# graphcore-research/bess-kge

Measured on AMD Instinct MI355X. Metric: positive+negative triples scored/sec, higher is better.
Workload: dtype f32; 1 GPU; ogbl-biokg-shaped ComplEx d=256 fp32 (W=512), 93,773 entities per shard, n_shard=1, S=4096 positives x 256 per-triple negatives per GPU per step, EmbeddingMoving, mode=score (gather+score+loss); negatives_per_triple=256, mode=score, collectives=none

## Files before the change

bess-kge_amd/csrc/neg_pertriple.hip:

```cpp
#include "common.h"
#include "loss_rows.h"

namespace bess {

struct NegPtArgs {
    const float* query;
    const void* base;
    const int32_t* idx;
    int64_t n_query;
    int n_neg;
    int W;
    int nch;
    int nb;
    int items_per_query;
    float sign;
    int accum = 0;
    float p = 2.f;
    int dn_by_row = 0;
    int sweep_shift = -1;
};

struct FuseArgs {
    const float* pos;
    int kind;
    float beta;
    float margin;
    float shift;
    float* st_ml;
    float* st_acc;
    const uint8_t* mask = nullptr;
    int64_t mask_rows = 0;
    int mask_cols = 0, mask_from = 0;
};

__device__ __forceinline__ float sigmoid_f(float x) { return 1.f / (1.f + expf(-x)); }

template <typename T, int VEC, int IT, int RED, int UNROLL, bool FUSE>
__global__ __launch_bounds__(256) void k_neg_pertriple_fwd(NegPtArgs a, float* __restrict__ out,
                                                           int64_t ld_out, FuseArgs f) {
    const int lane = threadIdx.x & 63;
    const int g = lane & 15;
    const int sub = lane >> 4;
    const int64_t item = blockIdx.x * 4ll + (threadIdx.x >> 6);
    if (item >= a.n_query * a.items_per_query) return;
    const int64_t q = item / a.items_per_query;
    const int k0 = static_cast<int>(item - q * a.items_per_query) * a.nb;
    const int k1 = min(k0 + a.nb, a.n_neg);

    float qv[IT][VEC];
    const float* qp = a.query + q * a.W;
#pragma unroll
    for (int it = 0; it < IT; ++it) {
        load_chunk<float, VEC>(qp, g + 16 * it, a.nch, qv[it]);
    }

    const T* base = static_cast<const T*>(a.base);
    const int32_t* idx = a.idx + q * a.n_neg;
    float* orow = out + q * ld_out;
    float fm = -INFINITY, fl = 0.f, facc[IT][VEC];
    float fpos = 0.f;
    if (FUSE) {
#pragma unroll
        for (int it = 0; it < IT; ++it)
#pragma unroll
            for (int v = 0; v < VEC; ++v) facc[it][v] = 0.f;
        if (f.kind == BESS_LOSS_MARGIN) fpos = f.pos[q];
    }

    int32_t nrow[UNROLL];
#pragma unroll
    for (int u = 0; u < UNROLL; ++u) nrow[u] = idx[min(k0 + sub + 4 * u, k1 - 1)];
    for (int kb = k0; kb < k1; kb += 4 * UNROLL) {
        float ev[UNROLL][IT][VEC];
        bool valid[UNROLL];
#pragma unroll
        for (int u = 0; u < UNROLL; ++u) {
            const int k = kb + sub + 4 * u;
            valid[u] = k < k1;
            const T* rp = base + static_cast<int64_t>(nrow[u]) * a.W;
            nrow[u] = idx[min(k + 4 * UNROLL, k1 - 1)];
#pragma unroll
            for (int it = 0; it < IT; ++it) {
                load_chunk<T, VEC>(rp, g + 16 * it, a.nch, ev[u][it]);
            }
        }
#pragma unroll
        for (int u = 0; u < UNROLL; ++u) {
            float acc = 0.f;
#pragma unroll
            for (int it = 0; it < IT; ++it) {
#pragma unroll
                for (int v = 0; v < VEC; ++v) {
                    if (RED == RED_DOT) {
                        acc = fmaf(qv[it][v], ev[u][it][v], acc);
                    } else if (RED == RED_L1) {
                        acc += fabsf(qv[it][v] - ev[u][it][v]);
                    } else {
                        acc += lp_term(qv[it][v] - ev[u][it][v], a.p);
                    }
                }
            }
            acc = row16_allreduce_sum(acc);
            if (RED == RED_L2) acc = lp_root(acc, a.p);
            float sc = a.sign * acc;
            if (FUSE && f.mask && valid[u]) {
                const int kcol = kb + sub + 4 * u - f.mask_from;
                const int64_t mrow = f.mask_rows == 1 ? 0 : q;
                if (kcol >= 0 && f.mask[mrow * f.mask_cols + kcol] == 0) sc += BESS_BAD_NEGATIVE_SCORE;
            }
            if (g == 0 && valid[u]) orow[kb + sub + 4 * u] = a.accum ? orow[kb + sub + 4 * u] + sc : sc;
            if (FUSE && valid[u]) {
                const float z = f.beta * (sc + f.shift);
                const float m_new = fmaxf(fm, z);
                const float corr = expf(fm - m_new);
                const float e = expf(z - m_new);
                float gs = 1.f;
                if (f.kind == BESS_LOSS_LOGSIGMOID) gs = sigmoid_f(sc + f.margin);
                else if (f.kind == BESS_LOSS_MARGIN) gs = (sc - fpos + f.margin > 0.f) ? 1.f : 0.f;
                const float p = e * gs;
                fl = fmaf(fl, corr, e);
                fm = m_new;
                const float inv_norm = RED == RED_L2 ? lp_inv(acc, a.p) : 0.f;
#pragma unroll
                for (int it = 0; it < IT; ++it)
#pragma unroll
                    for (int v = 0; v < VEC; ++v) {
                        float dsdq;
                        if (RED == RED_DOT) dsdq = ev[u][it][v];
                        else if (RED == RED_L1) dsdq = -sgnf(qv[it][v] - ev[u][it][v]);
                        else dsdq = -lp_dterm(qv[it][v] - ev[u][it][v], a.p) * inv_norm;
                        facc[it][v] = fmaf(facc[it][v], corr, p * dsdq);
                    }
            }
        }
    }
    if (FUSE) {
        float m_all = fmaxf(fm, __shfl_xor(fm, 16, 64));
        m_all = fmaxf(m_all, __shfl_xor(m_all, 32, 64));
        const float sc = (fm == -INFINITY) ? 0.f : expf(fm - m_all);
        float l = fl * sc;
        l += __shfl_xor(l, 16, 64);
        l += __shfl_xor(l, 32, 64);
        const int64_t slot = q * a.items_per_query + (item - q * a.items_per_query);
        if (lane == 0) {
            f.st_ml[slot * 2 + 0] = m_all;
            f.st_ml[slot * 2 + 1] = l;
        }
        float* ap = f.st_acc + slot * a.W;
#pragma unroll
        for (int it = 0; it < IT; ++it) {
            const int c = g + 16 * it;
#pragma unroll
            for (int v = 0; v < VEC; ++v) {
                float x = facc[it][v] * sc;
                x += __shfl_xor(x, 16, 64);
                x += __shfl_xor(x, 32, 64);
                if (sub == 0 && c < a.nch) ap[c * VEC + v] = x;
            }
        }
    }
}

constexpr int SW_NB = 1024;
constexpr int SW_PMAX = 8192;
constexpr int SW_PPT = SW_PMAX / 256;
constexpr int SW_SHARE = SW_PMAX / 8;
constexpr int SW_QFLOATS = 16384;
constexpr int64_t SW_REUSE_MIN = 4;

struct SweepArgs {
    int qb;
    int kc;
    int n_kchunks;
    int shift;
    int qstride;
};

template <typename T, int VEC, int IT, int RED, int UNROLL>
__global__ __launch_bounds__(256) void k_neg_pertriple_fwd_sweep(NegPtArgs a, SweepArgs s, float* __restrict__ out,
                                                                 int64_t ld_out) {
    extern __shared__ __attribute__((aligned(16))) float qs[];
    __shared__ int hist[SW_NB + 4];
    __shared__ int2 ent[SW_SHARE];
    __shared__ int rk[2][SW_PPT * 4];
    __shared__ int wsum[4];
    __shared__ int cut[4];

    const int tid = threadIdx.x;
    const int lane = tid & 63;
    const int wave = tid >> 6;
    const int label = blockIdx.x & 7;
    const int bc = blockIdx.x >> 3;
    const int qblk = bc / s.n_kchunks;
    const int kch = bc - qblk * s.n_kchunks;
    const int64_t q0 = static_cast<int64_t>(qblk) * s.qb;
    const int nqb = static_cast<int>(min(static_cast<int64_t>(s.qb), a.n_query - q0));
    const int kc0 = kch * s.kc;
    const int kcn = min(s.kc, a.n_neg - kc0);
    const int P = nqb * kcn;
    const int lo = static_cast<int>((static_cast<int64_t>(label) * P) >> 3);
    const int hi = static_cast<int>((static_cast<int64_t>(label + 1) * P) >> 3);

    for (int i = tid; i < nqb * IT * 16; i += 256) {
        const int qi = i / (IT * 16);
        const int c = i - qi * (IT * 16);
        float v[VEC];
        load_chunk<float, VEC>(a.query + (q0 + qi) * a.W, c, a.nch, v);
#pragma unroll
        for (int j = 0; j < VEC; ++j) qs[qi * s.qstride + c * VEC + j] = v[j];
    }
    for (int b = tid; b < SW_NB; b += 256) hist[b] = 0;
    if (tid < 2) cut[tid] = -1;
    int rr[SW_PPT];
#pragma unroll
    for (int j = 0; j < SW_PPT; ++j) {
        const int p = tid + 256 * j;
        rr[j] = 0;
        if (p < P) {
            const int qi = p / kcn;
            rr[j] = a.idx[(q0 + qi) * a.n_neg + kc0 + (p - qi * kcn)];
        }
    }
    __syncthreads();
#pragma unroll
    for (int j = 0; j < SW_PPT; ++j)
        if (tid + 256 * j < P) atomicAdd(&hist[min(static_cast<unsigned>(rr[j]) >> s.shift, SW_NB - 1u)], 1);
    __syncthreads();

    {
        int c[4], sum = 0;
#pragma unroll
        for (int i = 0; i < 4; ++i) {
            c[i] = hist[4 * tid + i];
            sum += c[i];
        }
        int incl = sum;
#pragma unroll
        for (int off = 1; off < 64; off <<= 1) {
            const int y = __shfl_up(incl, off, 64);
            if (lane >= off) incl += y;
        }
        if (lane == 63) wsum[wave] = incl;
        __syncthreads();
        int run = incl - sum;
        for (int w = 0; w < wave; ++w) run += wsum[w];
#pragma unroll
        for (int i = 0; i < 4; ++i) {
            const int b = 4 * tid + i;
            hist[b] = run;
            if (run < lo && lo < run + c[i]) cut[0] = b;
            if (run < hi && hi < run + c[i]) cut[1] = b;
            run += c[i];
        }
        if (tid == 255) hist[SW_NB] = run;
    }
    __syncthreads();

    const int cut0 = cut[0], cut1 = cut[1];
    const uint64_t lt = (1ull << lane) - 1ull;
#pragma unroll
    for (int j = 0; j < SW_PPT; ++j) {
        const bool live = tid + 256 * j < P;
        const unsigned b = min(static_cast<unsigned>(rr[j]) >> s.shift, SW_NB - 1u);
        const uint64_t m0 = __ballot(live && static_cast<int>(b) == cut0);
        const uint64_t m1 = __ballot(live && static_cast<int>(b) == cut1);
        if (lane == 0) {
            rk[0][j * 4 + wave] = __popcll(m0);
            rk[1][j * 4 + wave] = __popcll(m1);
        }
    }
    __syncthreads();
    if (wave == 0) {
#pragma unroll
        for (int h = 0; h < 2; ++h) {
            const int x0 = rk[h][2 * lane], x1 = rk[h][2 * lane + 1];
            int incl = x0 + x1;
#pragma unroll
            for (int off = 1; off < 64; off <<= 1) {
                const int y = __shfl_up(incl, off, 64);
                if (lane >= off) incl += y;
            }
            rk[h][2 * lane] = incl - x0 - x1;
            rk[h][2 * lane + 1] = incl - x1;
        }
    }
    __syncthreads();

    int slot[SW_PPT];
#pragma unroll
    for (int j = 0; j < SW_PPT; ++j) {
        const bool live = tid + 256 * j < P;
        const unsigned b = min(static_cast<unsigned>(rr[j]) >> s.shift, SW_NB - 1u);
        const bool in0 = live && static_cast<int>(b) == cut0;
        const bool in1 = live && static_cast<int>(b) == cut1 && !in0;
        const uint64_t m0 = __ballot(in0);
        const uint64_t m1 = __ballot(in1);
        const int b0 = live ? hist[b] : 0, b1 = live ? hist[b + 1] : 0;
        slot[j] = -1;
        if (live) {
            if (in0 || in1) {
                const int r = in0 ? rk[0][j * 4 + wave] + __popcll(m0 & lt) : rk[1][j * 4 + wave] + __popcll(m1 & lt);
                const int pos = b0 + r;
                if (pos >= lo && pos < hi) slot[j] = pos - lo;
            } else if (b0 >= lo && b1 <= hi) {
                slot[j] = -2;
            }
        }
    }
    __syncthreads();
#pragma unroll
    for (int j = 0; j < SW_PPT; ++j) {
        const int p = tid + 256 * j;
        if (slot[j] == -1) continue;
        const unsigned b = min(static_cast<unsigned>(rr[j]) >> s.shift, SW_NB - 1u);
        const int e = slot[j] >= 0 ? slot[j] : atomicAdd(&hist[b], 1) - lo;
        const int qi = p / kcn;
        ent[e] = make_int2(rr[j], (qi << 16) | (p - qi * kcn));
    }
    __syncthreads();

    const int n = hi - lo;
    const int g = lane & 15;
    const int sub = lane >> 4;
    const T* base = static_cast<const T*>(a.base);
    int2 nx[UNROLL];
#pragma unroll
    for (int u = 0; u < UNROLL; ++u) nx[u] = ent[max(0, min(wave * 4 * UNROLL + sub + 4 * u, n - 1))];
    for (int e0 = wave * 4 * UNROLL; e0 < n; e0 += 16 * UNROLL) {
        float ev[UNROLL][IT][VEC];
        int2 cur[UNROLL];
        bool valid[UNROLL];
#pragma unroll
        for (int u = 0; u < UNROLL; ++u) {
            const int e = e0 + sub + 4 * u;
            valid[u] = e < n;
            cur[u] = nx[u];
            const T* rp = base + static_cast<int64_t>(cur[u].x) * a.W;
            nx[u] = ent[min(e + 16 * UNROLL, n - 1)];
#pragma unroll
            for (int it = 0; it < IT; ++it) load_chunk<T, VEC>(rp, g + 16 * it, a.nch, ev[u][it]);
        }
#pragma unroll
        for (int u = 0; u < UNROLL; ++u) {
            const int qi = cur[u].y >> 16;
            const int kk = cur[u].y & 0xffff;
            const float* qp = qs + qi * s.qstride;
            float acc = 0.f;
#pragma unroll
            for (int it = 0; it < IT; ++it) {
                float qv[VEC];
                VecLoad<float, VEC>::load(qp + (g + 16 * it) * VEC, qv);
#pragma unroll
                for (int v = 0; v < VEC; ++v) {
                    if (RED == RED_DOT) {
                        acc = fmaf(qv[v], ev[u][it][v], acc);
                    } else if (RED == RED_L1) {
                        acc += fabsf(qv[v] - ev[u][it][v]);
                    } else {
                        acc += lp_term(qv[v] - ev[u][it][v], a.p);
                    }
                }
            }
            acc = row16_allreduce_sum(acc);
            if (RED == RED_L2) acc = lp_root(acc, a.p);
            if (g == 0 && valid[u]) out[(q0 + qi) * ld_out + kc0 + kk] = a.sign * acc;
        }
    }
}

__global__ __launch_bounds__(256) void k_combine_dq(const float* __restrict__ st_ml, const float* __restrict__ st_acc,
                                                    int64_t n_query, int items, int W, int kind, float loss_scale,
                                                    const float* __restrict__ pos, const float* __restrict__ weight,
                                                    int64_t weight_len, const float* __restrict__ norm,
                                                    float* __restrict__ d_query) {
    const int64_t q = blockIdx.x * 4ll + (threadIdx.x >> 6);
    if (q >= n_query) return;
    combine_dq_row(st_ml, st_acc, q, items, W, kind, loss_scale, pos, weight, weight_len, norm, d_query + q * W, nullptr);
}

template <typename T, int VEC, int IT, int RED, int UNROLL>
__global__ __launch_bounds__(256) void k_neg_pertriple_bwd(NegPtArgs a,
                                                           const float* __restrict__ d_out,
                                                           int64_t ld_dout,
                                                           float* __restrict__ d_query,
                                                           float* __restrict__ d_neg) {
    const int lane = threadIdx.x & 63;
    const int g = lane & 15;
    const int sub = lane >> 4;
    const int64_t item = blockIdx.x * 4ll + (threadIdx.x >> 6);
    if (item >= a.n_query * a.items_per_query) return;
    const int64_t q = item / a.items_per_query;
    const int k0 = static_cast<int>(item - q * a.items_per_query) * a.nb;
    const int k1 = min(k0 + a.nb, a.n_neg);

    float qv[IT][VEC], dq[IT][VEC];
    const float* qp = a.query + q * a.W;
#pragma unroll
    for (int it = 0; it < IT; ++it) {
#pragma unroll
        for (int v = 0; v < VEC; ++v) dq[it][v] = 0.f;
        load_chunk<float, VEC>(qp, g + 16 * it, a.nch, qv[it]);
    }
    const T* base = static_cast<const T*>(a.base);
    const int32_t* idx = a.idx + q * a.n_neg;
    const float* grow = d_out + q * ld_dout;

    int32_t nrow[UNROLL];
    float ngo[UNROLL];
#pragma unroll
    for (int u = 0; u < UNROLL; ++u) {
        const int kk = min(k0 + sub + 4 * u, k1 - 1);
        nrow[u] = idx[kk];
        ngo[u] = grow[kk];
    }
    const bool need_rows = !(RED == RED_DOT && d_query == nullptr);
    for (int kb = k0; kb < k1; kb += 4 * UNROLL) {
        float ev[UNROLL][IT][VEC], go[UNROLL];
        int ks[UNROLL];
        int32_t row_now[UNROLL];
        bool valid[UNROLL];
#pragma unroll
        for (int u = 0; u < UNROLL; ++u) {
            const int k = kb + sub + 4 * u;
            valid[u] = k < k1;
            ks[u] = min(k, k1 - 1);
            const T* rp = base + static_cast<int64_t>(nrow[u]) * a.W;
            row_now[u] = nrow[u];
            go[u] = valid[u] ? a.sign * ngo[u] : 0.f;
            const int kn = min(k + 4 * UNROLL, k1 - 1);
            nrow[u] = idx[kn];
            ngo[u] = grow[kn];
            if (need_rows) {
#pragma unroll
                for (int it = 0; it < IT; ++it) load_chunk<T, VEC>(rp, g + 16 * it, a.nch, ev[u][it]);
            } else {
#pragma unroll
                for (int it = 0; it < IT; ++it)
#pragma unroll
                    for (int v = 0; v < VEC; ++v) ev[u][it][v] = 0.f;
            }
        }
#pragma unroll
        for (int u = 0; u < UNROLL; ++u) {
            float gg = go[u];
            if (RED == RED_L2) {
                float ss = 0.f;
#pragma unroll
                for (int it = 0; it < IT; ++it)
#pragma unroll
                    for (int v = 0; v < VEC; ++v) {
                        ss += lp_term(qv[it][v] - ev[u][it][v], a.p);
                    }
                ss = row16_allreduce_sum(ss);
                gg *= lp_inv(lp_root(ss, a.p), a.p);
            }
            float* dn = d_neg + (a.dn_by_row ? static_cast<int64_t>(row_now[u]) : q * a.n_neg + ks[u]) * a.W;
#pragma unroll
            for (int it = 0; it < IT; ++it) {
                const int c = g + 16 * it;
                float de[VEC];
#pragma unroll
                for (int v = 0; v < VEC; ++v) {
                    float dqe;
                    if (RED == RED_DOT) {
                        dqe = gg * ev[u][it][v];
                        de[v] = gg * qv[it][v];
                    } else if (RED == RED_L1) {
                        dqe = gg * sgnf(qv[it][v] - ev[u][it][v]);
                        de[v] = -dqe;
                    } else {
                        dqe = gg * lp_dterm(qv[it][v] - ev[u][it][v], a.p);
                        de[v] = -dqe;
                    }
                    dq[it][v] += dqe;
                }
                if (d_neg && valid[u] && c < a.nch) {
                    if constexpr (VEC == 4) {
                        typedef float f4 __attribute__((ext_vector_type(4)));
#pragma unroll
                        for (int v = 0; v < VEC; v += 4) {
                            f4 o = {de[v], de[v + 1], de[v + 2], de[v + 3]};
                            __builtin_nontemporal_store(o, reinterpret_cast<f4*>(dn + c * VEC + v));
                        }
                    } else {
#pragma unroll
                        for (int v = 0; v < VEC; ++v) dn[c * VEC + v] = de[v];
                    }
                }
            }
        }
    }
    if (!d_query) return;
    float* dqp = d_query + q * a.W;
#pragma unroll
    for (int it = 0; it < IT; ++it) {
        const int c = g + 16 * it;
#pragma unroll
        for (int v = 0; v < VEC; ++v) {
            float x = dq[it][v];
            x += __shfl_xor(x, 16, 64);
            x += __shfl_xor(x, 32, 64);
            if (sub == 0 && c < a.nch) {
                if (a.items_per_query == 1) dqp[c * VEC + v] = x;
                else unsafeAtomicAdd(dqp + c * VEC + v, x);
            }
        }
    }
}

template <typename T, int VEC, int IT, int RED>
static void launch_fwd(const NegPtArgs& a, float* out, int64_t ld, const FuseArgs* fuse, hipStream_t st) {
    const int64_t items = a.n_query * a.items_per_query;
    constexpr int EPL = IT * VEC;
    constexpr int UNROLL = EPL <= 16 ? 4 : (EPL <= 32 ? 2 : 1);
    if (!fuse && a.sweep_shift >= 0) {
        SweepArgs s;
        s.qstride = IT * 16 * VEC;
        s.qb = SW_QFLOATS / s.qstride < 32 ? SW_QFLOATS / s.qstride : 32;
        s.kc = a.n_neg < SW_PMAX / s.qb ? a.n_neg : SW_PMAX / s.qb;
        s.n_kchunks = static_cast<int>(ceil_div(a.n_neg, s.kc));
        s.shift = a.sweep_shift;
        const int64_t blocks = ceil_div(a.n_query, s.qb) * s.n_kchunks * 8;
        const int lds = s.qb * s.qstride * static_cast<int>(sizeof(float));
        k_neg_pertriple_fwd_sweep<T, VEC, IT, RED, UNROLL>
            <<<static_cast<unsigned>(blocks), 256, lds, st>>>(a, s, out, ld);
    } else if (fuse) {
        constexpr int FU = EPL <= 16 ? 2 : 1;
        k_neg_pertriple_fwd<T, VEC, IT, RED, FU, true><<<ceil_div(items, 4), 256, 0, st>>>(a, out, ld, *fuse);
    } else {
        k_neg_pertriple_fwd<T, VEC, IT, RED, UNROLL, false><<<ceil_div(items, 4), 256, 0, st>>>(a, out, ld, FuseArgs{});
    }
}
template <typename T, int VEC, int IT, int RED>
static void launch_bwd(const NegPtArgs& a, const float* d_out, int64_t ld, float* dq, float* dn,
                       hipStream_t st) {
    const int64_t items = a.n_query * a.items_per_query;
    constexpr int EPL = IT * VEC;
    constexpr int BU = EPL <= 16 ? 2 : 1;
    k_neg_pertriple_bwd<T, VEC, IT, RED, BU><<<ceil_div(items, 4), 256, 0, st>>>(a, d_out, ld, dq, dn);
}

template <typename T, int VEC, int IT>
static void by_red(int red, bool fwd, const NegPtArgs& a, float* out, const float* d_out, int64_t ld,
                   float* dq, float* dn, const FuseArgs* fuse, hipStream_t st) {
    switch (red) {
        case RED_DOT:
            fwd ? launch_fwd<T, VEC, IT, RED_DOT>(a, out, ld, fuse, st)
                : launch_bwd<T, VEC, IT, RED_DOT>(a, d_out, ld, dq, dn, st);
            break;
        case RED_L1:
            fwd ? launch_fwd<T, VEC, IT, RED_L1>(a, out, ld, fuse, st)
                : launch_bwd<T, VEC, IT, RED_L1>(a, d_out, ld, dq, dn, st);
            break;
        default:
            fwd ? launch_fwd<T, VEC, IT, RED_L2>(a, out, ld, fuse, st)
                : launch_bwd<T, VEC, IT, RED_L2>(a, d_out, ld, dq, dn, st);
    }
}

template <typename T, int VEC>
static int by_it(int it, int red, bool fwd, const NegPtArgs& a, float* out, const float* d_out,
                 int64_t ld, float* dq, float* dn, const FuseArgs* fuse, hipStream_t st) {
    if (it <= 1) by_red<T, VEC, 1>(red, fwd, a, out, d_out, ld, dq, dn, fuse, st);
    else if (it <= 2) by_red<T, VEC, 2>(red, fwd, a, out, d_out, ld, dq, dn, fuse, st);
    else if (it <= 4) by_red<T, VEC, 4>(red, fwd, a, out, d_out, ld, dq, dn, fuse, st);
    else if (it <= 8) by_red<T, VEC, 8>(red, fwd, a, out, d_out, ld, dq, dn, fuse, st);
    else if (it <= 16) by_red<T, VEC, 16>(red, fwd, a, out, d_out, ld, dq, dn, fuse, st);
    else return fail(BESS_EUNSUPPORTED, "neg_score_pertriple: row of %d scalars too wide", a.W);
    return BESS_OK;
}

static int negatives_per_item(int64_t n_query, int64_t n_neg, int64_t row_bytes) {
    int nb = 64;
    while (nb < 256 && nb * row_bytes < 131072) nb <<= 1;
    while (nb > 8 && n_query * ceil_div(n_neg, nb) < 256 * 16 * 2) nb >>= 1;
    return nb;
}

static int vec_of(const bess_model_desc* d) {
    const int maxvec = d->dtype == BESS_F32 ? 4 : 8;
    if (d->width % maxvec == 0) return maxvec;
    return (d->dtype == BESS_F16 && d->width % 2 == 0) ? 2 : 1;
}

static int sweep_shift_for(const bess_model_desc* d, int64_t n_query, int64_t n_neg) {
    if (d->scorer > BESS_COMPLEX || d->width > 16 * 16 * vec_of(d)) return -1;
    const int64_t rows = d->reserved[1];
    if (rows <= 0 || n_query <= 0 || n_neg <= 0 || n_query * n_neg < SW_REUSE_MIN * rows) return -1;
    if (ceil_div(n_query, 8) * ceil_div(n_neg, 256) * 8 >= (1ll << 31)) return -1;
    int shift = 0;
    while (((rows - 1) >> shift) >= SW_NB) ++shift;
    return shift;
}

static int run(const bess_model_desc* d, bool fwd, const float* query, int64_t n_query,
               const void* neg_base, const int32_t* neg_idx, int64_t n_neg, float* out,
               const float* d_out, int64_t ld, float* dq, float* dn, void* stream,
               const FuseArgs* fuse = nullptr) {
    if (int e = check_desc(d)) return e;
    BESS_REQUIRE(n_query >= 0 && n_neg >= 0 && n_neg < (1ll << 31), "neg_score_pertriple: bad sizes");
    if (n_query == 0 || n_neg == 0) return BESS_OK;
    BESS_REQUIRE(query && neg_base && neg_idx, "neg_score_pertriple: NULL pointer");
    BESS_REQUIRE(ld >= n_neg, "neg_score_pertriple: leading dimension %lld < n_neg %lld", (long long)ld,
                 (long long)n_neg);
    if (d->scorer == BESS_BOXE)
        return boxe_negatives(d, fwd, false, query, n_query, neg_base, neg_idx, n_neg, out, d_out, ld, dq, dn,
                              as_stream(stream));
    if (d->scorer == BESS_AFFINE)
        return affine_pertriple(d, fwd, query, n_query, neg_base, neg_idx, n_neg, out, d_out, ld, dq, dn,
                                as_stream(stream));
    const int W = d->width;
    const int vec = vec_of(d);
    NegPtArgs a;
    a.query = query;
    a.base = neg_base;
    a.idx = neg_idx;
    a.n_query = n_query;
    a.n_neg = static_cast<int>(n_neg);
    a.W = W;
    a.nch = W / vec;
    a.nb = negatives_per_item(n_query, n_neg, static_cast<int64_t>(W) * (d->dtype == BESS_F32 ? 4 : 2));
    a.items_per_query = static_cast<int>(ceil_div(n_neg, a.nb));
    a.sign = is_distance(d->scorer) ? -1.f : 1.f;
    a.p = static_cast<float>(d->norm_p);
    a.dn_by_row = (!fwd && (d->reserved[0] & BESS_FLAG_DNEG_BY_ROW)) ? 1 : 0;
    if (fwd && !fuse) a.sweep_shift = sweep_shift_for(d, n_query, n_neg);
    const int red = reduce_of(d);
    hipStream_t st = as_stream(stream);
    if (!fwd && a.items_per_query > 1 && dq) {
        hipError_t e = fill_words_async(dq, 0u, n_query * W, st);
        if (e != hipSuccess) return fail(static_cast<int>(e), "memset d_query: %s", hipGetErrorString(e));
    }
    const int max_cols = 16 * 16 * vec;
    if (W > max_cols) {
        if (red == RED_L2)
            return fail(BESS_EUNSUPPORTED, "neg_score_pertriple: p = 2 on rows of %d scalars (more than %d)", W, max_cols);
        if (fuse)
            return fail(BESS_EUNSUPPORTED, "neg_score_pertriple: fused training forward on rows of %d scalars (more than %d)",
                        W, max_cols);
    }
    const int64_t sz = d->dtype == BESS_F32 ? 4 : 2;
    for (int col0 = 0; col0 < W; col0 += max_cols) {
        const int cols = W - col0 < max_cols ? W - col0 : max_cols;
        NegPtArgs w = a;
        w.query = query + col0;
        w.base = static_cast<const char*>(neg_base) + col0 * sz;
        w.nch = cols / vec;
        w.accum = col0 > 0;
        const int it = static_cast<int>(ceil_div(w.nch, 16));
        float* dqw = dq ? dq + col0 : nullptr;
        float* dnw = dn ? dn + col0 : nullptr;
        int rc = BESS_OK;
        if (d->dtype == BESS_F32) {
            if (vec == 4) rc = by_it<float, 4>(it, red, fwd, w, out, d_out, ld, dqw, dnw, fuse, st);
            else rc = by_it<float, 1>(it, red, fwd, w, out, d_out, ld, dqw, dnw, fuse, st);
        } else {
            if (vec == 8) rc = by_it<half_t, 8>(it, red, fwd, w, out, d_out, ld, dqw, dnw, fuse, st);
            else if (vec == 2) rc = by_it<half_t, 2>(it, red, fwd, w, out, d_out, ld, dqw, dnw, fuse, st);
            else rc = by_it<half_t, 1>(it, red, fwd, w, out, d_out, ld, dqw, dnw, fuse, st);
        }
        if (rc) return rc;
    }
    return check_launch(fwd ? "neg_score_pertriple_fwd" : "neg_score_pertriple_bwd");
}

}

extern "C" int bess_neg_score_pertriple_fwd(const bess_model_desc* d, const float* query,
                                            int64_t n_query, const void* neg_base,
                                            const int32_t* neg_idx, int64_t n_neg, float* out,
                                            int64_t ld_out, void* stream) {
    if (n_query > 0 && n_neg > 0 && !out) return bess::fail(BESS_EINVAL, "neg_score_pertriple_fwd: NULL out");
    return bess::run(d, true, query, n_query, neg_base, neg_idx, n_neg, out, nullptr, ld_out, nullptr,
                     nullptr, stream);
}

extern "C" int bess_neg_score_pertriple_bwd(const bess_model_desc* d, const float* query,
                                            int64_t n_query, const void* neg_base,
                                            const int32_t* neg_idx, int64_t n_neg,
                                            const float* d_out, int64_t ld_dout, float* d_query,
                                            float* d_neg, void* stream) {
    if (n_query > 0 && n_neg > 0 && !(d_out && (d_query || d_neg)))
        return bess::fail(BESS_EINVAL, "neg_score_pertriple_bwd: NULL pointer");
    return bess::run(d, false, query, n_query, neg_base, neg_idx, n_neg, nullptr, d_out, ld_dout,
                     d_query, d_neg, stream);
}

extern "C" int bess_neg_pertriple_sweep(const bess_model_desc* d, int64_t n_query, int64_t n_neg, int32_t* sweep) {
    if (int e = bess::check_desc(d)) return e;
    if (!sweep || n_query < 0 || n_neg < 0) return bess::fail(BESS_EINVAL, "neg_pertriple_sweep: bad argument");
    *sweep = bess::sweep_shift_for(d, n_query, n_neg) >= 0 ? 1 : 0;
    return BESS_OK;
}

static int64_t row_bytes_of(const bess_model_desc* d) {
    return static_cast<int64_t>(d->width) * (d->dtype == BESS_F32 ? 4 : 2);
}

extern "C" int bess_neg_pertriple_items(const bess_model_desc* d, int64_t n_query, int64_t n_neg, int32_t* items) {
    if (!d || !items || n_query < 0 || n_neg < 0) return bess::fail(BESS_EINVAL, "neg_pertriple_items: bad argument");
    *items = n_neg > 0 ? static_cast<int32_t>(bess::ceil_div(n_neg, bess::negatives_per_item(n_query, n_neg, row_bytes_of(d))))
                       : 0;
    return BESS_OK;
}

extern "C" int bess_neg_score_pertriple_fwd_dq(const bess_model_desc* d, const bess_loss_desc* l, const float* query,
                                               int64_t n_query, const void* neg_base, const int32_t* neg_idx,
                                               int64_t n_neg, const float* pos, const float* weight,
                                               int64_t weight_len, float* out, int64_t ld_out, float* d_query,
                                               float* state_ml, float* state_acc, void* stream) {
    return bess_neg_score_pertriple_fwd_dq_masked(d, l, query, n_query, neg_base, neg_idx, n_neg, pos, weight, weight_len,
                                                  nullptr, 0, 0, out, ld_out, d_query, state_ml, state_acc, stream);
}

extern "C" int bess_neg_score_pertriple_fwd_dq_masked(const bess_model_desc* d, const bess_loss_desc* l,
                                                      const float* query, int64_t n_query, const void* neg_base,
                                                      const int32_t* neg_idx, int64_t n_neg, const float* pos,
                                                      const float* weight, int64_t weight_len, const uint8_t* mask,
                                                      int64_t mask_rows, int64_t mask_cols, float* out,
                                                      int64_t ld_out, float* d_query, float* state_ml,
                                                      float* state_acc, void* stream) {
    using namespace bess;
    if (int e = check_desc(d)) return e;
    BESS_REQUIRE(l, "neg_score_pertriple_fwd_dq: NULL loss descriptor");
    BESS_REQUIRE(d->scorer <= BESS_COMPLEX, "neg_score_pertriple_fwd_dq: scorer %d has no fused form", d->scorer);
    BESS_REQUIRE(l->kind == BESS_LOSS_LOGSIGMOID || l->kind == BESS_LOSS_MARGIN || l->kind == BESS_LOSS_SSCE,
                 "neg_score_pertriple_fwd_dq: unknown loss %d", l->kind);
    if (n_query <= 0 || n_neg <= 0) return BESS_OK;
    BESS_REQUIRE(out && state_ml && state_acc && weight && (weight_len == 1 || weight_len == n_query),
                 "neg_score_pertriple_fwd_dq: NULL pointer or bad weight length");
    BESS_REQUIRE(pos || l->kind == BESS_LOSS_LOGSIGMOID, "neg_score_pertriple_fwd_dq: this loss needs the positive scores");
    FuseArgs f;
    f.pos = pos;
    f.kind = l->kind;
    f.beta = l->kind == BESS_LOSS_SSCE ? 1.f : (l->adversarial ? l->adversarial_scale : 0.f);
    f.margin = l->margin;
    f.shift = l->kind == BESS_LOSS_SSCE ? l->ssce_shift : 0.f;
    f.st_ml = state_ml;
    f.st_acc = state_acc;
    if (mask) {
        BESS_REQUIRE(mask_cols > 0 && mask_cols <= n_neg && (mask_rows == 1 || mask_rows == n_query),
                     "neg_score_pertriple_fwd_dq_masked: mask [%lld, %lld] for %lld queries x %lld negatives",
                     (long long)mask_rows, (long long)mask_cols, (long long)n_query, (long long)n_neg);
        f.mask = mask;
        f.mask_rows = mask_rows;
        f.mask_cols = static_cast<int>(mask_cols);
        f.mask_from = static_cast<int>(n_neg - mask_cols);
    }
    const int rc = run(d, true, query, n_query, neg_base, neg_idx, n_neg, out, nullptr, ld_out, nullptr, nullptr, stream,
                       &f);
    if (rc) return rc;
    const int items = static_cast<int>(ceil_div(n_neg, negatives_per_item(n_query, n_neg, row_bytes_of(d))));
    if (!d_query) return BESS_OK;
    k_combine_dq<<<static_cast<unsigned>(ceil_div(n_query, 4)), 256, 0, as_stream(stream)>>>(
        state_ml, state_acc, n_query, items, d->width, l->kind, l->loss_scale, pos, weight, weight_len, nullptr, d_query);
    return check_launch("neg_score_pertriple_fwd_dq");
}

extern "C" int bess_neg_score_pertriple_fwd_partials(const bess_model_desc* d, const bess_loss_desc* l,
                                                     const float* query, int64_t n_query, const void* neg_base,
                                                     const int32_t* neg_idx, int64_t n_neg, float* out,
                                                     int64_t ld_out, float* state_ml, float* state_acc, void* stream) {
    using namespace bess;
    if (int e = check_desc(d)) return e;
    BESS_REQUIRE(l, "neg_score_pertriple_fwd_partials: NULL loss descriptor");
    BESS_REQUIRE(d->scorer <= BESS_COMPLEX, "neg_score_pertriple_fwd_partials: scorer %d has no fused form", d->scorer);
    if (l->kind != BESS_LOSS_LOGSIGMOID && l->kind != BESS_LOSS_SSCE)
        return fail(BESS_EUNSUPPORTED, "neg_score_pertriple_fwd_partials: loss %d weighs a negative by the positive score, "
                                       "which the scoring shard does not have", l->kind);
    if (n_query <= 0 || n_neg <= 0) return BESS_OK;
    BESS_REQUIRE(out && state_ml && state_acc, "neg_score_pertriple_fwd_partials: NULL pointer");
    FuseArgs f;
    f.pos = nullptr;
    f.kind = l->kind;
    f.beta = l->kind == BESS_LOSS_SSCE ? 1.f : (l->adversarial ? l->adversarial_scale : 0.f);
    f.margin = l->margin;
    f.shift = l->kind == BESS_LOSS_SSCE ? l->ssce_shift : 0.f;
    f.st_ml = state_ml;
    f.st_acc = state_acc;
    return run(d, true, query, n_query, neg_base, neg_idx, n_neg, out, nullptr, ld_out, nullptr, nullptr, stream, &f);
}

extern "C" int bess_combine_dq_partials(const float* state_ml, const float* state_acc, int64_t n_query, int32_t items,
                                        int32_t width, const float* norm, float* d_query, void* stream) {
    using namespace bess;
    BESS_REQUIRE(n_query >= 0 && items > 0 && width > 0, "combine_dq_partials: bad sizes");
    if (n_query == 0) return BESS_OK;
    BESS_REQUIRE(state_ml && state_acc && norm && d_query, "combine_dq_partials: NULL pointer");
    k_combine_dq<<<static_cast<unsigned>(ceil_div(n_query, 4)), 256, 0, as_stream(stream)>>>(
        state_ml, state_acc, n_query, items, width, 0, 1.f, nullptr, nullptr, 1, norm, d_query);
    return check_launch("combine_dq_partials");
}
```

Before: 5.172 billion triples/s.

## Make row-sorted sweep kernel persistent with 512 threads and shared L2 position hint

```diff
diff --git a/bess-kge_amd/csrc/neg_pertriple.hip b/bess-kge_amd/csrc/neg_pertriple.hip
--- a/bess-kge_amd/csrc/neg_pertriple.hip
+++ b/bess-kge_amd/csrc/neg_pertriple.hip
@@ -163,208 +163,302 @@
 
 constexpr int SW_NB = 1024;
 constexpr int SW_PMAX = 8192;
-constexpr int SW_PPT = SW_PMAX / 256;
+constexpr int SW_NT = 512;
+constexpr int SW_NW = SW_NT / 64;
+constexpr int SW_PPT = SW_PMAX / SW_NT;
+constexpr int SW_BPT = SW_NB / SW_NT;
 constexpr int SW_SHARE = SW_PMAX / 8;
 constexpr int SW_QFLOATS = 16384;
 constexpr int64_t SW_REUSE_MIN = 4;
+constexpr int SW_HINT_EVERY = 4;
+
+__device__ int sw_hint[8 * 32];
 
 struct SweepArgs {
     int qb;
     int kc;
     int n_kchunks;
+    int n_bc;
     int shift;
     int qstride;
 };
 
+#ifdef BESS_SWEEP_TRACE
+constexpr int SW_TRACE_WORDS = 24;
+static unsigned long long* g_sweep_trace = nullptr;
+static long long g_sweep_trace_records = 0;
+#define SW_TRACE_PARAMS , unsigned long long *trace, long long trace_records
+#define SW_TRACE_ARGS , g_sweep_trace, g_sweep_trace_records
+#else
+#define SW_TRACE_PARAMS
+#define SW_TRACE_ARGS
+#endif
+
 template <typename T, int VEC, int IT, int RED, int UNROLL>
-__global__ __launch_bounds__(256) void k_neg_pertriple_fwd_sweep(NegPtArgs a, SweepArgs s, float* __restrict__ out,
-                                                                 int64_t ld_out) {
+__global__ __launch_bounds__(SW_NT, (VEC > 1 && IT <= 8 ? 4 : 2)) void k_neg_pertriple_fwd_sweep(
+    NegPtArgs a, SweepArgs s, float* __restrict__ out, int64_t ld_out SW_TRACE_PARAMS) {
     extern __shared__ __attribute__((aligned(16))) float qs[];
     __shared__ int hist[SW_NB + 4];
     __shared__ int2 ent[SW_SHARE];
-    __shared__ int rk[2][SW_PPT * 4];
-    __shared__ int wsum[4];
+    __shared__ int rk[2][SW_PMAX / 64];
+    __shared__ int wsum[SW_NW];
     __shared__ int cut[4];
 
     const int tid = threadIdx.x;
     const int lane = tid & 63;
     const int wave = tid >> 6;
+    const int g = lane & 15;
+    const int sub = lane >> 4;
+    const T* base = static_cast<const T*>(a.base);
     const int label = blockIdx.x & 7;
-    const int bc = blockIdx.x >> 3;
-    const int qblk = bc / s.n_kchunks;
-    const int kch = bc - qblk * s.n_kchunks;
-    const int64_t q0 = static_cast<int64_t>(qblk) * s.qb;
-    const int nqb = static_cast<int>(min(static_cast<int64_t>(s.qb), a.n_query - q0));
-    const int kc0 = kch * s.kc;
-    const int kcn = min(s.kc, a.n_neg - kc0);
-    const int P = nqb * kcn;
-    const int lo = static_cast<int>((static_cast<int64_t>(label) * P) >> 3);
-    const int hi = static_cast<int>((static_cast<int64_t>(label + 1) * P) >> 3);
-
-    for (int i = tid; i < nqb * IT * 16; i += 256) {
-        const int qi = i / (IT * 16);
-        const int c = i - qi * (IT * 16);
-        float v[VEC];
-        load_chunk<float, VEC>(a.query + (q0 + qi) * a.W, c, a.nch, v);
-#pragma unroll
-        for (int j = 0; j < VEC; ++j) qs[qi * s.qstride + c * VEC + j] = v[j];
-    }
-    for (int b = tid; b < SW_NB; b += 256) hist[b] = 0;
-    if (tid < 2) cut[tid] = -1;
-    int rr[SW_PPT];
-#pragma unroll
-    for (int j = 0; j < SW_PPT; ++j) {
-        const int p = tid + 256 * j;
-        rr[j] = 0;
-        if (p < P) {
-            const int qi = p / kcn;
-            rr[j] = a.idx[(q0 + qi) * a.n_neg + kc0 + (p - qi * kcn)];
-        }
-    }
-    __syncthreads();
-#pragma unroll
-    for (int j = 0; j < SW_PPT; ++j)
-        if (tid + 256 * j < P) atomicAdd(&hist[min(static_cast<unsigned>(rr[j]) >> s.shift, SW_NB - 1u)], 1);
-    __syncthreads();
-
-    {
-        int c[4], sum = 0;
-#pragma unroll
-        for (int i = 0; i < 4; ++i) {
-            c[i] = hist[4 * tid + i];
-            sum += c[i];
-        }
-        int incl = sum;
-#pragma unroll
-        for (int off = 1; off < 64; off <<= 1) {
-            const int y = __shfl_up(incl, off, 64);
-            if (lane >= off) incl += y;
-        }
-        if (lane == 63) wsum[wave] = incl;
+    const int bc_step = static_cast<int>(gridDim.x >> 3);
+#ifdef BESS_SWEEP_TRACE
+    int chunk_no = 0;
+#endif
+    for (int bc = blockIdx.x >> 3; bc < s.n_bc; bc += bc_step) {
+#ifdef BESS_SWEEP_TRACE
+        unsigned long long* rec = nullptr;
+        {
+            const long long r = static_cast<long long>(blockIdx.x) * ((s.n_bc + bc_step - 1) / bc_step) + chunk_no++;
+            if (trace && r < trace_records) rec = trace + r * SW_TRACE_WORDS;
+            if (rec && tid == 0) {
+                rec[0] = wall_clock64();
+                rec[3] = __builtin_amdgcn_s_getreg((3 << 11) | 20) & 15;
+                rec[5] = blockIdx.x;
+                rec[6] = bc;
+            }
+        }
+#endif
+        const int qblk = bc / s.n_kchunks;
+        const int kch = bc - qblk * s.n_kchunks;
+        const int64_t q0 = static_cast<int64_t>(qblk) * s.qb;
+        const int nqb = static_cast<int>(min(static_cast<int64_t>(s.qb), a.n_query - q0));
+        const int kc0 = kch * s.kc;
+        const int kcn = min(s.kc, a.n_neg - kc0);
+        const int P = nqb * kcn;
+        const int lo = static_cast<int>((static_cast<int64_t>(label) * P) >> 3);
+        const int hi = static_cast<int>((static_cast<int64_t>(label + 1) * P) >> 3);
+
+        for (int i = tid; i < nqb * IT * 16; i += SW_NT) {
+            const int qi = i / (IT * 16);
+            const int c = i - qi * (IT * 16);
+            float v[VEC];
+            load_chunk<float, VEC>(a.query + (q0 + qi) * a.W, c, a.nch, v);
+#pragma unroll
+            for (int j = 0; j < VEC; ++j) qs[qi * s.qstride + c * VEC + j] = v[j];
+        }
+        for (int b = tid; b < SW_NB; b += SW_NT) hist[b] = 0;
+        if (tid < 2) cut[tid] = -1;
+        if (tid == 2) cut[2] = __hip_atomic_load(&sw_hint[label * 32], __ATOMIC_RELAXED, __HIP_MEMORY_SCOPE_AGENT);
+        const int dqi = SW_NT / kcn, dkk = SW_NT - dqi * kcn;
+        const int qi0 = tid / kcn, kk0 = tid - qi0 * kcn;
+        int rr[SW_PPT];
+        {
+            int qi = qi0, kk = kk0;
+#pragma unroll
+            for (int j = 0; j < SW_PPT; ++j) {
+                rr[j] = tid + SW_NT * j < P ? a.idx[(q0 + qi) * a.n_neg + kc0 + kk] : 0;
+                qi += dqi;
+                kk += dkk;
+                if (kk >= kcn) {
+                    kk -= kcn;
+                    ++qi;
+                }
+            }
+        }
         __syncthreads();
-        int run = incl - sum;
-        for (int w = 0; w < wave; ++w) run += wsum[w];
-#pragma unroll
-        for (int i = 0; i < 4; ++i) {
-            const int b = 4 * tid + i;
-            hist[b] = run;
-            if (run < lo && lo < run + c[i]) cut[0] = b;
-            if (run < hi && hi < run + c[i]) cut[1] = b;
-            run += c[i];
-        }
-        if (tid == 255) hist[SW_NB] = run;
-    }
-    __syncthreads();
-
-    const int cut0 = cut[0], cut1 = cut[1];
-    const uint64_t lt = (1ull << lane) - 1ull;
-#pragma unroll
-    for (int j = 0; j < SW_PPT; ++j) {
-        const bool live = tid + 256 * j < P;
-        const unsigned b = min(static_cast<unsigned>(rr[j]) >> s.shift, SW_NB - 1u);
-        const uint64_t m0 = __ballot(live && static_cast<int>(b) == cut0);
-        const uint64_t m1 = __ballot(live && static_cast<int>(b) == cut1);
-        if (lane == 0) {
-            rk[0][j * 4 + wave] = __popcll(m0);
-            rk[1][j * 4 + wave] = __popcll(m1);
-        }
-    }
-    __syncthreads();
-    if (wave == 0) {
-#pragma unroll
-        for (int h = 0; h < 2; ++h) {
-            const int x0 = rk[h][2 * lane], x1 = rk[h][2 * lane + 1];
-            int incl = x0 + x1;
+#pragma unroll
+        for (int j = 0; j < SW_PPT; ++j)
+            if (tid + SW_NT * j < P) atomicAdd(&hist[min(static_cast<unsigned>(rr[j]) >> s.shift, SW_NB - 1u)], 1);
+        __syncthreads();
+
+        {
+            int c[SW_BPT], sum = 0;
+#pragma unroll
+            for (int i = 0; i < SW_BPT; ++i) {
+                c[i] = hist[SW_BPT * tid + i];
+                sum += c[i];
+            }
+            int incl = sum;
 #pragma unroll
             for (int off = 1; off < 64; off <<= 1) {
                 const int y = __shfl_up(incl, off, 64);
                 if (lane >= off) incl += y;
             }
-            rk[h][2 * lane] = incl - x0 - x1;
-            rk[h][2 * lane + 1] = incl - x1;
-        }
-    }
-    __syncthreads();
-
-    int slot[SW_PPT];
-#pragma unroll
-    for (int j = 0; j < SW_PPT; ++j) {
-        const bool live = tid + 256 * j < P;
-        const unsigned b = min(static_cast<unsigned>(rr[j]) >> s.shift, SW_NB - 1u);
-        const bool in0 = live && static_cast<int>(b) == cut0;
-        const bool in1 = live && static_cast<int>(b) == cut1 && !in0;
-        const uint64_t m0 = __ballot(in0);
-        const uint64_t m1 = __ballot(in1);
-        const int b0 = live ? hist[b] : 0, b1 = live ? hist[b + 1] : 0;
-        slot[j] = -1;
-        if (live) {
-            if (in0 || in1) {
-                const int r = in0 ? rk[0][j * 4 + wave] + __popcll(m0 & lt) : rk[1][j * 4 + wave] + __popcll(m1 & lt);
-                const int pos = b0 + r;
-                if (pos >= lo && pos < hi) slot[j] = pos - lo;
-            } else if (b0 >= lo && b1 <= hi) {
-                slot[j] = -2;
-            }
-        }
-    }
-    __syncthreads();
-#pragma unroll
-    for (int j = 0; j < SW_PPT; ++j) {
-        const int p = tid + 256 * j;
-        if (slot[j] == -1) continue;
-        const unsigned b = min(static_cast<unsigned>(rr[j]) >> s.shift, SW_NB - 1u);
-        const int e = slot[j] >= 0 ? slot[j] : atomicAdd(&hist[b], 1) - lo;
-        const int qi = p / kcn;
-        ent[e] = make_int2(rr[j], (qi << 16) | (p - qi * kcn));
-    }
-    __syncthreads();
-
-    const int n = hi - lo;
-    const int g = lane & 15;
-    const int sub = lane >> 4;
-    const T* base = static_cast<const T*>(a.base);
-    int2 nx[UNROLL];
-#pragma unroll
-    for (int u = 0; u < UNROLL; ++u) nx[u] = ent[max(0, min(wave * 4 * UNROLL + sub + 4 * u, n - 1))];
-    for (int e0 = wave * 4 * UNROLL; e0 < n; e0 += 16 * UNROLL) {
-        float ev[UNROLL][IT][VEC];
-        int2 cur[UNROLL];
-        bool valid[UNROLL];
+            if (lane == 63) wsum[wave] = incl;
+            __syncthreads();
+            int run = incl - sum;
+            for (int w = 0; w < wave; ++w) run += wsum[w];
+#pragma unroll
+            for (int i = 0; i < SW_BPT; ++i) {
+                const int b = SW_BPT * tid + i;
+                hist[b] = run;
+                if (run < lo && lo < run + c[i]) cut[0] = b;
+                if (run < hi && hi < run + c[i]) cut[1] = b;
+                run += c[i];
+            }
+            if (tid == SW_NT - 1) hist[SW_NB] = run;
+        }
+        __syncthreads();
+
+        const int cut0 = cut[0], cut1 = cut[1];
+#pragma unroll
+        for (int j = 0; j < SW_PPT; ++j) {
+            const bool live = tid + SW_NT * j < P;
+            const unsigned b = min(static_cast<unsigned>(rr[j]) >> s.shift, SW_NB - 1u);
+            const uint64_t m0 = __ballot(live && static_cast<int>(b) == cut0);
+            const uint64_t m1 = __ballot(live && static_cast<int>(b) == cut1);
+            if (lane == 0) {
+                rk[0][j * SW_NW + wave] = __popcll(m0);
+                rk[1][j * SW_NW + wave] = __popcll(m1);
+            }
+        }
+        __syncthreads();
+        if (wave == 0) {
+#pragma unroll
+            for (int h = 0; h < 2; ++h) {
+                const int x0 = rk[h][2 * lane], x1 = rk[h][2 * lane + 1];
+                int incl = x0 + x1;
+#pragma unroll
+                for (int off = 1; off < 64; off <<= 1) {
+                    const int y = __shfl_up(incl, off, 64);
+                    if (lane >= off) incl += y;
+                }
+                rk[h][2 * lane] = incl - x0 - x1;
+                rk[h][2 * lane + 1] = incl - x1;
+            }
+        }
+        __syncthreads();
+
+        const uint64_t lt = (1ull << lane) - 1ull;
+        int slot[SW_PPT];
+#pragma unroll
+        for (int j = 0; j < SW_PPT; ++j) {
+            const bool live = tid + SW_NT * j < P;
+            const unsigned b = min(static_cast<unsigned>(rr[j]) >> s.shift, SW_NB - 1u);
+            const bool in0 = live && static_cast<int>(b) == cut0;
+            const bool in1 = live && static_cast<int>(b) == cut1 && !in0;
+            const uint64_t m0 = __ballot(in0);
+            const uint64_t m1 = __ballot(in1);
+            const int b0 = live ? hist[b] : 0, b1 = live ? hist[b + 1] : 0;
+            slot[j] = -1;
+            if (live) {
+                if (in0 || in1) {
+                    const int r = in0 ? rk[0][j * SW_NW + wave] + __popcll(m0 & lt)
+                                      : rk[1][j * SW_NW + wave] + __popcll(m1 & lt);
+                    const int pos = b0 + r;
+                    if (pos >= lo && pos < hi) slot[j] = pos - lo;
+                } else if (b0 >= lo && b1 <= hi) {
+                    slot[j] = -2;
+                }
+            }
+        }
+        __syncthreads();
+        {
+            int qi = qi0, kk = kk0;
+#pragma unroll
+            for (int j = 0; j < SW_PPT; ++j) {
+                if (slot[j] != -1) {
+                    const unsigned b = min(static_cast<unsigned>(rr[j]) >> s.shift, SW_NB - 1u);
+                    const int e = slot[j] >= 0 ? slot[j] : atomicAdd(&hist[b], 1) - lo;
+                    ent[e] = make_int2(rr[j], (qi << 16) | kk);
+                }
+                qi += dqi;
+                kk += dkk;
+                if (kk >= kcn) {
+                    kk -= kcn;
+                    ++qi;
+                }
+            }
+        }
+        __syncthreads();
+
+        const int n = hi - lo;
+        int first = 0;
+        {
+            const int hb = cut[2];
+            int l = 0, r = n;
+            while (l < r) {
+                const int m = (l + r) >> 1;
+                if (static_cast<int>(min(static_cast<unsigned>(ent[m].x) >> s.shift, SW_NB - 1u)) < hb) l = m + 1;
+                else r = m;
+            }
+            first = l < n ? l : 0;
+        }
+#ifdef BESS_SWEEP_TRACE
+        if (rec && tid == 0) {
+            rec[1] = wall_clock64();
+            rec[4] = n > 0 ? min(static_cast<unsigned>(ent[first].x) >> s.shift, SW_NB - 1u) : 0;
+            rec[7] = n;
+        }
+        const int tr_iters = (n + SW_NW * 4 * UNROLL - 1) / (SW_NW * 4 * UNROLL);
+        const int tr_every = max(1, (tr_iters + 7) / 8);
+#endif
+
+        int2 nx[UNROLL];
 #pragma unroll
         for (int u = 0; u < UNROLL; ++u) {
-            const int e = e0 + sub + 4 * u;
-            valid[u] = e < n;
-            cur[u] = nx[u];
-            const T* rp = base + static_cast<int64_t>(cur[u].x) * a.W;
-            nx[u] = ent[min(e + 16 * UNROLL, n - 1)];
-#pragma unroll
-            for (int it = 0; it < IT; ++it) load_chunk<T, VEC>(rp, g + 16 * it, a.nch, ev[u][it]);
-        }
-#pragma unroll
-        for (int u = 0; u < UNROLL; ++u) {
-            const int qi = cur[u].y >> 16;
-            const int kk = cur[u].y & 0xffff;
-            const float* qp = qs + qi * s.qstride;
-            float acc = 0.f;
-#pragma unroll
-            for (int it = 0; it < IT; ++it) {
-                float qv[VEC];
-                VecLoad<float, VEC>::load(qp + (g + 16 * it) * VEC, qv);
-#pragma unroll
-                for (int v = 0; v < VEC; ++v) {
-                    if (RED == RED_DOT) {
-                        acc = fmaf(qv[v], ev[u][it][v], acc);
-                    } else if (RED == RED_L1) {
-                        acc += fabsf(qv[v] - ev[u][it][v]);
-                    } else {
-                        acc += lp_term(qv[v] - ev[u][it][v], a.p);
+            int e = max(0, min(wave * 4 * UNROLL + sub + 4 * u, n - 1)) + first;
+            if (e >= n) e -= n;
+            nx[u] = ent[max(e, 0)];
+        }
+        int iter = 0;
+        for (int e0 = wave * 4 * UNROLL; e0 < n; e0 += SW_NW * 4 * UNROLL, ++iter) {
+            float ev[UNROLL][IT][VEC];
+            int2 cur[UNROLL];
+            bool valid[UNROLL];
+#pragma unroll
+            for (int u = 0; u < UNROLL; ++u) {
+                const int e = e0 + sub + 4 * u;
+                valid[u] = e < n;
+                cur[u] = nx[u];
+                const T* rp = base + static_cast<int64_t>(cur[u].x) * a.W;
+                int en = min(e + SW_NW * 4 * UNROLL, n - 1) + first;
+                if (en >= n) en -= n;
+                nx[u] = ent[en];
+#pragma unroll
+                for (int it = 0; it < IT; ++it) load_chunk<T, VEC>(rp, g + 16 * it, a.nch, ev[u][it]);
+            }
+            if (tid == 0 && iter % SW_HINT_EVERY == 0)
+                __hip_atomic_store(&sw_hint[label * 32],
+                                   static_cast<int>(min(static_cast<unsigned>(cur[0].x) >> s.shift, SW_NB - 1u)),
+                                   __ATOMIC_RELAXED, __HIP_MEMORY_SCOPE_AGENT);
+#ifdef BESS_SWEEP_TRACE
+            if (rec && tid == 0 && iter % tr_every == 0 && iter / tr_every < 8) {
+                rec[8 + iter / tr_every] = wall_clock64();
+                rec[16 + iter / tr_every] = min(static_cast<unsigned>(cur[0].x) >> s.shift, SW_NB - 1u);
+            }
+#endif
+#pragma unroll
+            for (int u = 0; u < UNROLL; ++u) {
+                const int qi = cur[u].y >> 16;
+                const int kk = cur[u].y & 0xffff;
+                const float* qp = qs + qi * s.qstride;
+                float acc = 0.f;
+#pragma unroll
+                for (int it = 0; it < IT; ++it) {
+                    float qv[VEC];
+                    VecLoad<float, VEC>::load(qp + (g + 16 * it) * VEC, qv);
+#pragma unroll
+                    for (int v = 0; v < VEC; ++v) {
+                        if (RED == RED_DOT) {
+                            acc = fmaf(qv[v], ev[u][it][v], acc);
+                        } else if (RED == RED_L1) {
+                            acc += fabsf(qv[v] - ev[u][it][v]);
+                        } else {
+                            acc += lp_term(qv[v] - ev[u][it][v], a.p);
+                        }
                     }
                 }
-            }
-            acc = row16_allreduce_sum(acc);
-            if (RED == RED_L2) acc = lp_root(acc, a.p);
-            if (g == 0 && valid[u]) out[(q0 + qi) * ld_out + kc0 + kk] = a.sign * acc;
-        }
+                acc = row16_allreduce_sum(acc);
+                if (RED == RED_L2) acc = lp_root(acc, a.p);
+                if (g == 0 && valid[u]) out[(q0 + qi) * ld_out + kc0 + kk] = a.sign * acc;
+            }
+        }
+        __syncthreads();
+#ifdef BESS_SWEEP_TRACE
+        if (rec && tid == 0) rec[2] = wall_clock64();
+#endif
     }
 }
 
@@ -519,11 +613,24 @@
         s.qb = SW_QFLOATS / s.qstride < 32 ? SW_QFLOATS / s.qstride : 32;
         s.kc = a.n_neg < SW_PMAX / s.qb ? a.n_neg : SW_PMAX / s.qb;
         s.n_kchunks = static_cast<int>(ceil_div(a.n_neg, s.kc));
+        s.n_bc = static_cast<int>(ceil_div(a.n_query, s.qb) * s.n_kchunks);
         s.shift = a.sweep_shift;
-        const int64_t blocks = ceil_div(a.n_query, s.qb) * s.n_kchunks * 8;
         const int lds = s.qb * s.qstride * static_cast<int>(sizeof(float));
+        int64_t blocks = static_cast<int64_t>(s.n_bc) * 8;
+        static const int resident = [lds] {
+            int dev = 0, cus = 0, per_cu = 0;
+            if (hipGetDevice(&dev) != hipSuccess ||
+                hipDeviceGetAttribute(&cus, hipDeviceAttributeMultiprocessorCount, dev) != hipSuccess ||
+                hipOccupancyMaxActiveBlocksPerMultiprocessor(&per_cu, k_neg_pertriple_fwd_sweep<T, VEC, IT, RED, UNROLL>,
+                                                             SW_NT, lds) != hipSuccess) {
+                (void)hipGetLastError();
+                return 0;
+            }
+            return per_cu * cus / 8 * 8;
+        }();
+        if (resident >= 8 && resident < blocks) blocks = resident;
         k_neg_pertriple_fwd_sweep<T, VEC, IT, RED, UNROLL>
-            <<<static_cast<unsigned>(blocks), 256, lds, st>>>(a, s, out, ld);
+            <<<static_cast<unsigned>(blocks), SW_NT, lds, st>>>(a, s, out, ld SW_TRACE_ARGS);
     } else if (fuse) {
         constexpr int FU = EPL <= 16 ? 2 : 1;
         k_neg_pertriple_fwd<T, VEC, IT, RED, FU, true><<<ceil_div(items, 4), 256, 0, st>>>(a, out, ld, *fuse);
@@ -693,6 +800,14 @@
     return BESS_OK;
 }
 
+#ifdef BESS_SWEEP_TRACE
+extern "C" int bess_sweep_trace_buffer(void* buf, int64_t records) {
+    bess::g_sweep_trace = static_cast<unsigned long long*>(buf);
+    bess::g_sweep_trace_records = buf ? records : 0;
+    return BESS_OK;
+}
+#endif
+
 static int64_t row_bytes_of(const bess_model_desc* d) {
     return static_cast<int64_t>(d->width) * (d->dtype == BESS_F32 ? 4 : 2);
 }
diff --git a/profiles/trace_pertriple_sweep.py b/profiles/trace_pertriple_sweep.py
--- /dev/null
+++ b/profiles/trace_pertriple_sweep.py
@@ -0,0 +1,114 @@
+#!/usr/bin/env python3
+import argparse
+import ctypes
+import os
+import statistics
+import sys
+
+REPO = os.path.dirname(os.path.dirname(os.path.abspath(__file__)))
+sys.path[:0] = [os.path.join(REPO, "bess-kge_amd"), REPO]
+import numpy as np
+import torch
+
+from besskge import _native as nat
+
+WORDS = 24
+TICK_US = 0.01
+
+ap = argparse.ArgumentParser()
+ap.add_argument("--lib", default=os.path.join(REPO, "profiles", "probe_lib", "libbesskge_hip_trace.so"))
+ap.add_argument("--rows", type=int, default=93_773)
+args = ap.parse_args()
+if not os.path.exists(args.lib):
+    raise SystemExit(f"{args.lib} is missing: make -C bess-kge_amd/csrc SWEEP_TRACE=1")
+lib = ctypes.CDLL(args.lib)
+lib.bess_sweep_trace_buffer.argtypes = [ctypes.c_void_p, ctypes.c_int64]
+lib.bess_neg_score_pertriple_fwd.argtypes = ([ctypes.c_void_p] * 2 + [ctypes.c_int64] + [ctypes.c_void_p] * 2
+                                             + [ctypes.c_int64, ctypes.c_void_p, ctypes.c_int64, ctypes.c_void_p])
+
+dev = torch.device("cuda", 0)
+W, S, N = 512, 4096, 256
+torch.manual_seed(0)
+table = torch.randn(args.rows, W, device=dev) * 0.1
+q = torch.randn(S, W, device=dev)
+idx = torch.randint(args.rows, (S * N,), device=dev).to(torch.int32)
+out = torch.empty(S, N, device=dev)
+d = nat.with_row_count(nat.make_desc(nat.COMPLEX, 0, table, W), table)
+assert nat.pertriple_sweep(d, S, N), "the shape must take the row-ordered kernel"
+shift = 0
+while (args.rows - 1) >> shift >= 1024:
+    shift += 1
+
+
+def launch():
+    rc = lib.bess_neg_score_pertriple_fwd(ctypes.addressof(d), q.data_ptr(), S, table.data_ptr(), idx.data_ptr(), N,
+                                          out.data_ptr(), N, torch.cuda.current_stream().cuda_stream)
+    assert rc == 0, rc
+
+
+for _ in range(2):
+    launch()
+torch.cuda.synchronize()
+records = 1 << 14
+buf = torch.zeros(records * WORDS, dtype=torch.int64, device=dev)
+assert lib.bess_sweep_trace_buffer(buf.data_ptr(), records) == 0
+a, b = torch.cuda.Event(enable_timing=True), torch.cuda.Event(enable_timing=True)
+a.record()
+launch()
+b.record()
+torch.cuda.synchronize()
+lib.bess_sweep_trace_buffer(None, 0)
+r = buf.cpu().numpy().reshape(records, WORDS)
+r = r[r[:, 2] != 0]
+t_first = r[:, 0].min()
+t = lambda x: (x - t_first) * TICK_US
+life, pro = t(r[:, 2]) - t(r[:, 0]), t(r[:, 1]) - t(r[:, 0])
+span = t(r[:, 2].max())
+wgs = len(set(r[:, 5].tolist()))
+print(f"rows {args.rows:,d} (buckets of {1 << shift} rows)  launch {1e3 * a.elapsed_time(b):.1f} us by events, "
+      f"{span:.1f} us first entry to last exit; {wgs} workgroups, {len(r)} block chunks")
+print(f"prologue: {pro.mean():.2f} us of a chunk's {life.mean():.2f} us (share {pro.sum() / life.sum():.3f}; "
+      f"min {pro.min():.2f} max {pro.max():.2f} us)")
+print(f"chunk life: min {life.min():.1f} median {np.median(life):.1f} max {life.max():.1f} us")
+
+late = t(r[:, 0]) > 5.0
+mid = span / 2
+print(f"{'xcc':>3s} {'labels':>8s} {'chunks':>6s} {'late':>5s} | late starts: {'first':>7s} {'median':>7s} {'last':>7s} {'spread':>7s} us |"
+      f" buckets at {mid:.0f} us: {'min':>5s} {'median':>6s} {'max':>5s} {'spread':>6s} (of range)   first-entry buckets of late chunks")
+late_spreads, mid_spreads = [], []
+
+
+def ring_spread(pos, lo_b, rng):
+    p = sorted((x - lo_b) / (rng + 1) for x in pos)
+    gaps = [b - a for a, b in zip(p, p[1:])] + [p[0] + 1 - p[-1]]
+    return 1 - max(gaps)
+
+
+for x in sorted(set(r[:, 3].tolist())):
+    m = r[r[:, 3] == x]
+    ml = m[t(m[:, 0]) > 5.0]
+    labels = sorted(set((m[:, 5] & 7).tolist()))
+    pos = []
+    for rec in m:
+        if not (rec[1] <= t_first + mid / TICK_US <= rec[2]):
+            continue
+        stamps = [(rec[8 + k], rec[16 + k]) for k in range(8) if rec[8 + k]]
+        before = [s for s in stamps if t(s[0]) <= mid]
+        if before:
+            pos.append(before[-1][1])
+    lo_b = min(rec[16 + k] for rec in m for k in range(8) if rec[8 + k])
+    hi_b = max(rec[16 + k] for rec in m for k in range(8) if rec[8 + k])
+    rng = max(1, hi_b - lo_b)
+    ls = t(ml[:, 0]) if len(ml) else np.zeros(1)
+    late_spreads.append(ls.max() - ls.min())
+    if pos:
+        mid_spreads.append(ring_spread(pos, lo_b, rng))
+    fe = sorted(ml[:, 4].tolist())
+    fe_txt = f"{fe[0]}..{fe[len(fe) // 2]}..{fe[-1]}" if fe else "-"
+    print(f"{x:3d} {str(labels):>8s} {len(m):6d} {len(ml):5d} | {ls.min():20.1f} {np.median(ls):7.1f} {ls.max():7.1f} {ls.max() - ls.min():7.1f}    |"
+          + (f" {min(pos):17d} {int(statistics.median(pos)):6d} {max(pos):5d} {ring_spread(pos, lo_b, rng):6.2f} ({lo_b}-{hi_b})" if pos else " " * 45)
+          + f"   {fe_txt}")
+print(f"late-start spread within an XCD: mean {np.mean(late_spreads):.1f} us, max {np.max(late_spreads):.1f} us")
+if mid_spreads:
+    print(f"row positions of an XCD's workgroups at mid-kernel: spread {np.mean(mid_spreads):.2f} of the XCD's row range on "
+          f"average (max {np.max(mid_spreads):.2f}); one L2 holds {4 * 2 ** 20 / (args.rows / 8 * W * 4):.2f} of it")
```

Measured after the change: 5.072 billion triples/s. -1.9%, worse.
